# tensorlayer/TLXCV

Hardware: AMD Instinct MI355X
Metric: images/sec fwd (higher is better)
Workload: dtype f16; 1 GPU; ResNet-50 fp16 forward, 224x224, batch 256 per GPU (BASELINE configs[1]); global_batch=256, per_gpu_batch=256, weights=seeded random (tlxcv_amd.seeded, seed 1), parallelism=single GPU, launch=hipGraph replay of the forward

## Files before the change

tlxcv_amd/csrc/block_seam.hip:

```cpp
#include "kernel_util.h"
#include <stdio.h>
#include "block_seam.h"
#include <type_traits>
#ifdef TLXMI_TUNING
#define TLXMI_DBG_NT(x) (x)
#else
#define TLXMI_DBG_NT(x) (false)
#endif

namespace tlxmi {

static __device__ __forceinline__ int bs_f1(int r) { return ((r >> 1) & 1) | (((r >> 4) & 3) << 1); }
static __device__ __forceinline__ int bs_f2(int r) { return (((r >> 1) & 1) << 2) | ((r >> 5) & 1); }

static __device__ __forceinline__ unsigned bs_pkrelu(unsigned v) {
    unsigned r;
    asm("v_pk_max_f16 %0, %1, 0" : "=v"(r) : "v"(v));
    return r;
}
static __device__ __forceinline__ u32x2 bs_bn_skip_relu4(f32x4 acc, f32x4 sc, f32x4 sh, half4v skip) {
    f32x2 t0 = f32x2{__builtin_fmaf(acc[0], sc[0], (float)skip[0]), __builtin_fmaf(acc[1], sc[1], (float)skip[1])};
    f32x2 t1 = f32x2{__builtin_fmaf(acc[2], sc[2], (float)skip[2]), __builtin_fmaf(acc[3], sc[3], (float)skip[3])};
    t0 += f32x2{sh[0], sh[1]};
    t1 += f32x2{sh[2], sh[3]};
// ... 240 lines not shown
        for (int tt = 0; tt < T2; ++tt) {
            if (TLXMI_DBG(a, 16)) continue;
#pragma unroll
            for (int s = 0; s < 2; ++s) {
                const u32x4 af = *reinterpret_cast<const u32x4*>(wb + (CB + (tt >> 2)) * PANEL + (a2off[tt & 3] ^ (s << 4)));
#pragma unroll
                for (int pw = 0; pw < PW; ++pw) acc2[tt][pw] = Mma<half_t>::run(af, yf[pw][s], acc2[tt][pw]);
            }
        }

        if (more) {
            stage_write((c + 1) & 1, st);
#pragma unroll
            for (int pw = 0; pw < PW; ++pw) { sk[pw][0] = skn[pw][0]; sk[pw][1] = skn[pw][1]; }
        }
        __syncthreads();
    }

#pragma unroll
    for (int q = 0; q < N2 / 64; ++q) {
        const float* sc = tab1 + 64 * q + 16 * g;
        const float* sh = sc + N2;
#pragma unroll
        for (int h = 0; h < 2; ++h) {
            const f32x4 s0 = *reinterpret_cast<const f32x4*>(sc + 8 * h), s1 = *reinterpret_cast<const f32x4*>(sc + 8 * h + 4);
            const f32x4 h0 = *reinterpret_cast<const f32x4*>(sh + 8 * h), h1 = *reinterpret_cast<const f32x4*>(sh + 8 * h + 4);
#pragma unroll
            for (int pw = 0; pw < PW; ++pw) {
                u32x2 o0, o1;
                if constexpr (MLP) {
                    const half8v rv = __builtin_bit_cast(half8v, buf_load16(rsrd, pok[pw] ? (pix[pw] * a.res_ld + 64 * q + 16 * g + 8 * h) * 2 : BUF_OOB));
                    o0 = bs_bn_res4(acc2[4 * q + 2 * h][pw], s0, h0, half4v{rv[0], rv[1], rv[2], rv[3]});
                    o1 = bs_bn_res4(acc2[4 * q + 2 * h + 1][pw], s1, h1, half4v{rv[4], rv[5], rv[6], rv[7]});
                } else {
                    o0 = bs_bn_relu4(acc2[4 * q + 2 * h][pw], s0, h0);
                    o1 = bs_bn_relu4(acc2[4 * q + 2 * h + 1][pw], s1, h1);
                }
                const u32x4 o = u32x4{o0[0], o0[1], o1[0], o1[1]};
                if (TLXMI_DBG(a, 4)) continue;
                if (TLXMI_DBG_NT(a.z_nt)) buf_store16<BUF_NT>(zsrd, o, pok[pw] ? (pix[pw] * a.z_ld + 64 * q + 16 * g + 8 * h) * 2 : BUF_OOB);
                else buf_store16(zsrd, o, pok[pw] ? (pix[pw] * a.z_ld + 64 * q + 16 * g + 8 * h) * 2 : BUF_OOB);
            }
        }
    }
}

template <int K1, int N2, int NW>
__global__ __launch_bounds__(64 * NW, 1) void seam_pair_kernel(const SeamArgs a) {
    static_assert(N2 % 128 == 0 && NW % 2 == 0, "pairs of waves split N2 in halves of whole 64-channel blocks");
    constexpr int NT = 64 * NW;
    constexpr int IPT = 512 / NT;
    constexpr int PW = 2;
    constexpr int KS = K1 / 32;
    constexpr int CB = K1 / 64;
    constexpr int Q2 = N2 / 64;
    constexpr int NP = CB + Q2;
    constexpr int T2H = N2 / 32;
    constexpr int PANEL = 64 * 128;
    extern __shared__ __attribute__((aligned(16))) char smem[];
    char* const wbuf = smem;
    float* const tab3 = reinterpret_cast<float*>(smem + 2 * NP * PANEL);
    float* const tab1 = tab3 + 2 * a.N1;
    char* const ybuf = reinterpret_cast<char*>(tab1 + 2 * N2);

    const int t = threadIdx.x, lane = t & 63;
    const int wid = __builtin_amdgcn_readfirstlane(t >> 6);
    const int hh = wid & 1, pp = wid >> 1;
    const int fr = lane & 15, g = lane >> 4;

    const __amdgpu_buffer_rsrc_t xsrd = buf_srd(a.x, a.x_bytes), w3srd = buf_srd(a.w3, a.w3_bytes), w1srd = buf_srd(a.w1, a.w1_bytes);
    const __amdgpu_buffer_rsrc_t rsrd = buf_srd(a.res, a.res_bytes), ysrd = buf_srd(a.y, a.y_bytes), zsrd = buf_srd(a.z, a.z_bytes);

    auto stage_load = [&](int c, u32x4 (&st)[NP][IPT]) {
#pragma unroll
        for (int k = 0; k < IPT; ++k) {
            const int idx = k * NT + t, srow = idx >> 3, sslot = idx & 7;
            const int sl1 = sslot ^ bs_f1(srow), sl2 = sslot ^ bs_f2(srow);
#pragma unroll
            for (int cb = 0; cb < CB; ++cb) st[cb][k] = buf_load16(w3srd, ((64 * c + srow) * K1 + 64 * cb + 8 * sl1) * 2);
#pragma unroll
            for (int q = 0; q < Q2; ++q) st[CB + q][k] = buf_load16(w1srd, ((64 * q + srow) * a.N1 + 64 * c + 8 * sl2) * 2);
        }
    };
    auto stage_write = [&](int buf, const u32x4 (&st)[NP][IPT]) {
#pragma unroll
        for (int j = 0; j < NP; ++j)
#pragma unroll
            for (int k = 0; k < IPT; ++k) *reinterpret_cast<u32x4*>(wbuf + (buf * NP + j) * PANEL + (k * NT + t) * 16) = st[j][k];
    };

    const int m0 = ((int)blockIdx.x * (NW / 2) + pp) * (16 * PW);
    int pix[PW];
    bool pok[PW];
#pragma unroll
    for (int pw = 0; pw < PW; ++pw) {
        pix[pw] = m0 + 16 * pw + fr;
        pok[pw] = pix[pw] < a.M;
    }
    u32x4 xf[KS][PW];
#pragma unroll
    for (int pw = 0; pw < PW; ++pw)
#pragma unroll
        for (int ks = 0; ks < KS; ++ks)
            xf[ks][pw] = buf_load16(xsrd, pok[pw] ? (pix[pw] * a.x_ld + 32 * ks + 8 * g) * 2 : BUF_OOB);
    auto skip_load = [&](int c, u32x4 (&sk)[PW]) {
#pragma unroll
        for (int pw = 0; pw < PW; ++pw) sk[pw] = buf_load16(rsrd, pok[pw] ? (pix[pw] * a.res_ld + 64 * c + 16 * g + 8 * hh) * 2 : BUF_OOB);
    };
    u32x4 sk[PW];
    skip_load(0, sk);
    {
        u32x4 st[NP][IPT];
        stage_load(0, st);
        for (int i = t; i < a.N1; i += NT) {
            tab3[i] = a.scale3 ? a.scale3[i] : 1.f;
            tab3[a.N1 + i] = a.shift3 ? a.shift3[i] : 0.f;
        }
        for (int i = t; i < N2; i += NT) {
            tab1[i] = a.scale1 ? a.scale1[i] : 1.f;
            tab1[N2 + i] = a.shift1 ? a.shift1[i] : 0.f;
        }
        stage_write(0, st);
    }
    __syncthreads();

    const int arow = 16 * (fr >> 2) + (fr & 3);
    int a1off[2], a2off[4];
#pragma unroll
    for (int e = 0; e < 2; ++e) {
        const int r = arow + 4 * (2 * hh + e);
        a1off[e] = r * 128 + ((g ^ bs_f1(r)) << 4);
    }
#pragma unroll
    for (int ci = 0; ci < 4; ++ci) {
        const int r = arow + 4 * ci;
        a2off[ci] = r * 128 + (((2 * g) ^ bs_f2(r)) << 4);
    }
    char* const ymine = ybuf + (wid * PW * 64 + lane) * 16;
    const char* const ypart = ybuf + ((wid ^ 1) * PW * 64 + lane) * 16;

    f32x4 acc2[T2H][PW];
#pragma unroll
    for (int tt = 0; tt < T2H; ++tt)
#pragma unroll
        for (int pw = 0; pw < PW; ++pw) acc2[tt][pw] = f32x4{0.f, 0.f, 0.f, 0.f};

    const int nch = a.N1 >> 6;
#pragma unroll 1
    for (int c = 0; c < nch; ++c) {
        const char* const wb = wbuf + (c & 1) * NP * PANEL;
        const bool more = c + 1 < nch;
        u32x4 st[NP][IPT], skn[PW];
        if (more) {
            stage_load(c + 1, st);
            skip_load(c + 1, skn);
        }
        f32x4 acc1[2][PW];
#pragma unroll
        for (int e = 0; e < 2; ++e) {
#pragma unroll
            for (int pw = 0; pw < PW; ++pw) acc1[e][pw] = f32x4{0.f, 0.f, 0.f, 0.f};
#pragma unroll
            for (int ks = 0; ks < KS; ++ks) {
                const u32x4 af = *reinterpret_cast<const u32x4*>(wb + (ks >> 1) * PANEL + (a1off[e] ^ ((ks & 1) << 6)));
#pragma unroll
                for (int pw = 0; pw < PW; ++pw) acc1[e][pw] = Mma<half_t>::run(af, xf[ks][pw], acc1[e][pw]);
            }
        }
        u32x4 yf[PW][2];
        {
            const float* sc = tab3 + 64 * c + 16 * g + 8 * hh;
            const float* sh = sc + a.N1;
            const f32x4 s0 = *reinterpret_cast<const f32x4*>(sc), s1 = *reinterpret_cast<const f32x4*>(sc + 4);
            const f32x4 h0 = *reinterpret_cast<const f32x4*>(sh), h1 = *reinterpret_cast<const f32x4*>(sh + 4);
#pragma unroll
            for (int pw = 0; pw < PW; ++pw) {
                const half8v rv = __builtin_bit_cast(half8v, sk[pw]);
                const u32x2 o0 = bs_bn_skip_relu4(acc1[0][pw], s0, h0, half4v{rv[0], rv[1], rv[2], rv[3]});
                const u32x2 o1 = bs_bn_skip_relu4(acc1[1][pw], s1, h1, half4v{rv[4], rv[5], rv[6], rv[7]});
                const u32x4 o = u32x4{o0[0], o0[1], o1[0], o1[1]};
                buf_store16(ysrd, o, pok[pw] ? (pix[pw] * a.y_ld + 64 * c + 16 * g + 8 * hh) * 2 : BUF_OOB);
                *reinterpret_cast<u32x4*>(ymine + pw * 1024) = o;
                if (hh == 0) yf[pw][0] = o; else yf[pw][1] = o;
            }
        }
        __syncthreads();
#pragma unroll
        for (int pw = 0; pw < PW; ++pw) {
            const u32x4 o = *reinterpret_cast<const u32x4*>(ypart + pw * 1024);
            if (hh == 0) yf[pw][1] = o; else yf[pw][0] = o;
        }
#pragma unroll
        for (int tt = 0; tt < T2H; ++tt) {
#pragma unroll
            for (int s = 0; s < 2; ++s) {
                const u32x4 af = *reinterpret_cast<const u32x4*>(wb + (CB + hh * (Q2 / 2) + (tt >> 2)) * PANEL + (a2off[tt & 3] ^ (s << 4)));
#pragma unroll
                for (int pw = 0; pw < PW; ++pw) acc2[tt][pw] = Mma<half_t>::run(af, yf[pw][s], acc2[tt][pw]);
            }
        }
        if (more) {
            stage_write((c + 1) & 1, st);
#pragma unroll
            for (int pw = 0; pw < PW; ++pw) sk[pw] = skn[pw];
        }
        __syncthreads();
    }

#pragma unroll
    for (int q = 0; q < Q2 / 2; ++q) {
        const float* sc = tab1 + 64 * (hh * (Q2 / 2) + q) + 16 * g;
        const float* sh = sc + N2;
#pragma unroll
        for (int h = 0; h < 2; ++h) {
            const f32x4 s0 = *reinterpret_cast<const f32x4*>(sc + 8 * h), s1 = *reinterpret_cast<const f32x4*>(sc + 8 * h + 4);
            const f32x4 h0 = *reinterpret_cast<const f32x4*>(sh + 8 * h), h1 = *reinterpret_cast<const f32x4*>(sh + 8 * h + 4);
#pragma unroll
            for (int pw = 0; pw < PW; ++pw) {
                const u32x2 o0 = bs_bn_relu4(acc2[4 * q + 2 * h][pw], s0, h0), o1 = bs_bn_relu4(acc2[4 * q + 2 * h + 1][pw], s1, h1);
                const u32x4 o = u32x4{o0[0], o0[1], o1[0], o1[1]};
                buf_store16(zsrd, o, pok[pw] ? (pix[pw] * a.z_ld + 64 * (hh * (Q2 / 2) + q) + 16 * g + 8 * h) * 2 : BUF_OOB);
            }
        }
    }
}

template <int K1, int N2, int NW> static int launch_seam_pair_t(const SeamArgs& a, hipStream_t st) {
    constexpr int NP = K1 / 64 + N2 / 64;
    const size_t lds = (size_t)2 * NP * 64 * 128 + (size_t)(2 * a.N1 + 2 * N2) * sizeof(float) + (size_t)NW * 2 * 1024;
    if (lds > 160 * 1024) return fail(TLXMI_ERR_UNSUPPORTED, "block_seam: %zu bytes of LDS", lds);
    const void* fn = reinterpret_cast<const void*>(&seam_pair_kernel<K1, N2, NW>);
    if (int rc = raise_lds_limit(fn, 160 * 1024, "block_seam")) return rc;
    const long grid = ((long)a.M + NW * 16 - 1) / (NW * 16);
    if (grid >= (1l << 31)) return fail(TLXMI_ERR_UNSUPPORTED, "block_seam: too many rows");
    SeamArgs b = a;
    void* args[] = {&b};
    hipError_t e = hipLaunchKernel(fn, dim3((unsigned)grid), dim3(64 * NW), args, lds, st);
    if (e != hipSuccess) return fail(TLXMI_ERR_LAUNCH, "block_seam: HIP launch failed: %s", hipGetErrorString(e));
    return TLXMI_OK;
}

template <int K1, int N2, int PW, int NW, bool PROJ = false, int WPS = 0, bool MLP = false, bool DEC = false>
static int launch_seam_t(const std::conditional_t<DEC, SeamDecArgs, SeamArgs>& a, hipStream_t st) {
    constexpr int NP = K1 / 64 + N2 / 64 + (PROJ ? K1 / 64 : 0);
    const size_t lds = (size_t)2 * NP * 64 * 128 + (size_t)(2 * a.N1 + 2 * N2 + (PROJ ? 2 * a.N1 : 0)) * sizeof(float);
    if (lds > 160 * 1024) return fail(TLXMI_ERR_UNSUPPORTED, "block_seam: %zu bytes of LDS", lds);
    const void* fn = reinterpret_cast<const void*>(&seam_kernel<K1, N2, PW, NW, PROJ, WPS, MLP, DEC>);
    if (lds > 64 * 1024)
        if (int rc = raise_lds_limit(fn, 160 * 1024, "block_seam")) return rc;
    const long grid = ((long)a.M + NW * 16 * PW - 1) / (NW * 16 * PW);
    if (grid >= (1l << 31)) return fail(TLXMI_ERR_UNSUPPORTED, "block_seam: too many rows");
#ifdef TLXMI_TUNING
    if (tune_int("TLXMI_SEAM_OCC", 0)) {
        int nb = -1;
        hipError_t oe = hipOccupancyMaxActiveBlocksPerMultiprocessor(&nb, fn, 64 * NW, lds);
        fprintf(stderr, "seam<%d,%d,%d,%d,%d>: lds %zu, grid %ld, occupancy %d workgroups / CU (%s)\n", K1, N2, PW, NW, (int)PROJ, lds, grid, nb, hipGetErrorString(oe));
    }
#endif
    auto b = a;
    void* args[] = {&b};
    hipError_t e = hipLaunchKernel(fn, dim3((unsigned)grid), dim3(64 * NW), args, lds, st);
    if (e != hipSuccess) return fail(TLXMI_ERR_LAUNCH, "block_seam: HIP launch failed: %s", hipGetErrorString(e));
    return TLXMI_OK;
}

bool block_seam_shape_ok(int K1, int N1, int N2) {
    if (N1 % 64 || N1 < 64 || N1 > 2048) return false;
    if (!((K1 == 64 && (N2 == 64 || N2 == 128)) || (K1 == 128 && (N2 == 128 || N2 == 256)) || (K1 == 256 && N2 == 256))) return false;
    const size_t lds = (size_t)2 * (K1 / 64 + N2 / 64) * 64 * 128 + (size_t)(2 * N1 + 2 * N2) * sizeof(float) + (K1 == 256 ? (size_t)8 * 2 * 1024 : 0);
    return lds <= 160 * 1024;
}

int launch_mlp_seam(const SeamArgs& a0, int K1, int N2, hipStream_t st) {
    SeamArgs b = a0;
    b.z_nt = b.y_nt = 0;
    b.debug = 0;
    if (K1 == 128 && N2 == 128) return launch_seam_t<128, 128, 2, 8, false, 0, true>(b, st);
    return fail(TLXMI_ERR_UNSUPPORTED, "mlp_seam: no instantiation for %d -> N1 -> %d channels", K1, N2);
}

int launch_block_seam(const SeamArgs& a0, int K1, int N2, hipStream_t st) {
    const int vv = (int)tune_int("TLXMI_SEAM", 0);
    const int v = vv & 1;
    SeamArgs b = a0;
    b.z_nt = (vv & 2) ? 1 : 0;
    b.y_nt = (vv & 4) ? 1 : 0;
    b.debug = (int)tune_int("TLXMI_SEAM_DBG", 0);
    const SeamArgs& a = b;
    if (a.wd) {
        if (K1 == 64 && N2 == 64) return launch_seam_t<64, 64, 2, 4, true>(a, st);
        return fail(TLXMI_ERR_UNSUPPORTED, "block_seam: the projection-shortcut form is compiled for 64 -> N1 -> 64 channels");
    }
    if (vv & 16) {
        if (K1 == 64 && N2 == 64) return launch_seam_t<64, 64, 2, 4, false, 3>(a, st);
        if (K1 == 64 && N2 == 128) return launch_seam_t<64, 128, 2, 4, false, 3>(a, st);
        if (K1 == 128 && N2 == 128) return launch_seam_t<128, 128, 2, 4, false, 2>(a, st);
    }
    if (K1 == 64 && N2 == 64) return v ? launch_seam_t<64, 64, 2, 8>(a, st) : launch_seam_t<64, 64, 2, 4>(a, st);
    if (K1 == 64 && N2 == 128) return v ? launch_seam_t<64, 128, 2, 8>(a, st) : launch_seam_t<64, 128, 2, 4>(a, st);
    if (K1 == 128 && N2 == 128) return v ? launch_seam_t<128, 128, 2, 4>(a, st) : launch_seam_t<128, 128, 2, 8>(a, st);
    if (K1 == 128 && N2 == 256) return v ? launch_seam_t<128, 256, 1, 4>(a, st) : launch_seam_t<128, 256, 1, 8>(a, st);
    if (K1 == 256 && N2 == 256) {
        if (!(vv & 32)) return launch_seam_pair_t<256, 256, 8>(a, st);
        return v ? launch_seam_t<256, 256, 1, 4>(a, st) : launch_seam_t<256, 256, 1, 8>(a, st);
    }
    return fail(TLXMI_ERR_UNSUPPORTED, "block_seam: no instantiation for %d -> N1 -> %d channels", K1, N2);
}

static bool block_seam_dec_shape_ok(int K1, int N1, int N2) {
    return ((K1 == 64 && N1 == 256 && N2 == 128) || (K1 == 128 && N1 == 512 && N2 == 256)) && block_seam_shape_ok(K1, N1, N2);
}

int launch_block_seam_dec(const SeamDecArgs& a0, int K1, int N2, hipStream_t st) {
    SeamDecArgs b = a0;
    b.z_nt = b.y_nt = 0;
    b.debug = 0;
    if (K1 == 64 && N2 == 128) return launch_seam_t<64, 128, 2, 4, false, 0, false, true>(b, st);
    if (K1 == 128 && N2 == 256) return launch_seam_t<128, 256, 1, 8, false, 0, false, true>(b, st);
    return fail(TLXMI_ERR_UNSUPPORTED, "block_seam_dec: no instantiation for %d -> N1 -> %d channels", K1, N2);
}

}

using namespace tlxmi;

extern "C" int tlxmi_bottleneck_seam_supported(int dtype, int K1, int N1, int N2) {
    return dtype == TLXMI_F16 && block_seam_shape_ok(K1, N1, N2) ? 1 : 0;
}

static int seam_impl(const tlxmi_seam_desc* d, const void* t2, const void* w3_packed, const float* scale3,
                     const float* shift3, const void* skip, void* y, const void* w1_packed, const float* scale1,
                     const float* shift1, void* t1, void* stream, const void* wd_packed, const float* scale_d, const float* shift_d) {
    TLXMI_REQUIRE(d && t2 && w3_packed && skip && y && w1_packed && t1, TLXMI_ERR_BAD_ARG, "bottleneck_seam: null argument");
    TLXMI_REQUIRE(d->dtype == TLXMI_F16, TLXMI_ERR_UNSUPPORTED, "bottleneck_seam: fp16 only (the fp32 parity mode runs the two convolutions)");
    TLXMI_REQUIRE(d->rows > 0 && d->K1 > 0 && d->N1 > 0 && d->N2 > 0, TLXMI_ERR_BAD_ARG, "bottleneck_seam: bad extent");
    if (!block_seam_shape_ok(d->K1, d->N1, d->N2))
        return fail(TLXMI_ERR_UNSUPPORTED, "bottleneck_seam: no kernel for %d -> %d -> %d channels", d->K1, d->N1, d->N2);
    TLXMI_REQUIRE(d->t2_ld >= d->K1 && d->skip_ld >= (wd_packed ? d->K1 : d->N1) && d->y_ld >= d->N1 && d->t1_ld >= d->N2, TLXMI_ERR_BAD_ARG, "bottleneck_seam: row stride below the channel count");
    TLXMI_REQUIRE(!wd_packed || (aligned16(wd_packed) && d->K1 == 64 && d->N2 == 64), TLXMI_ERR_UNSUPPORTED, "bottleneck_seam_proj: 64 -> N1 -> 64 channels only");
    TLXMI_REQUIRE(d->t2_ld % 8 == 0 && d->skip_ld % 8 == 0 && d->y_ld % 8 == 0 && d->t1_ld % 8 == 0 && aligned16(t2) && aligned16(skip) && aligned16(y) &&
                      aligned16(t1) && aligned16(w3_packed) && aligned16(w1_packed),
                  TLXMI_ERR_ALIGNMENT, "bottleneck_seam: rows must be whole 16-byte chunks");
    TLXMI_REQUIRE(d->act == TLXMI_ACT_RELU, TLXMI_ERR_UNSUPPORTED, "bottleneck_seam: ReLU after both convolutions only");
    const long long rows = d->rows;
    const long long big = (1ll << 31);
    TLXMI_REQUIRE(rows * d->t2_ld * 2 < big && rows * d->skip_ld * 2 < big && rows * d->y_ld * 2 < big && rows * d->t1_ld * 2 < big && rows < big,
                  TLXMI_ERR_UNSUPPORTED, "bottleneck_seam: a tensor exceeds the 2 GiB the 32-bit buffer offsets address");
    SeamArgs a;
    a.x = (const char*)t2; a.w3 = (const char*)w3_packed; a.res = (const char*)skip; a.w1 = (const char*)w1_packed;
    a.y = (char*)y; a.z = (char*)t1;
    a.scale3 = scale3; a.shift3 = shift3; a.scale1 = scale1; a.shift1 = shift1;
    a.M = (int)rows; a.N1 = d->N1;
    a.x_ld = d->t2_ld; a.res_ld = d->skip_ld; a.y_ld = d->y_ld; a.z_ld = d->t1_ld;
    a.x_bytes = (unsigned)(rows * d->t2_ld * 2); a.res_bytes = (unsigned)(rows * d->skip_ld * 2);
    a.y_bytes = (unsigned)(rows * d->y_ld * 2); a.z_bytes = (unsigned)(rows * d->t1_ld * 2);
    a.wd = (const char*)wd_packed; a.scale_d = scale_d; a.shift_d = shift_d;
    a.wd_bytes = wd_packed ? (unsigned)(((size_t)(d->N1 + 127) / 128 * 128) * (size_t)d->K1 * 2) : 0u;
    a.w3_bytes = (unsigned)(((size_t)(d->N1 + 127) / 128 * 128) * (size_t)d->K1 * 2);
    a.w1_bytes = (unsigned)(((size_t)(d->N2 + 127) / 128 * 128) * (size_t)d->N1 * 2);
    const int rc = launch_block_seam(a, d->K1, d->N2, as_stream(stream));
    if (rc != TLXMI_OK) return rc;
    return check_launch("bottleneck_seam");
}

extern "C" int tlxmi_bottleneck_seam(const tlxmi_seam_desc* d, const void* t2, const void* w3_packed, const float* scale3,
                                     const float* shift3, const void* skip, void* y, const void* w1_packed, const float* scale1,
                                     const float* shift1, void* t1, void* stream) {
    return seam_impl(d, t2, w3_packed, scale3, shift3, skip, y, w1_packed, scale1, shift1, t1, stream, nullptr, nullptr, nullptr);
}

extern "C" int tlxmi_bottleneck_seam_proj(const tlxmi_seam_desc* d, const void* t2, const void* w3_packed, const float* scale3,
                                          const float* shift3, const void* x, const void* wd_packed, const float* scale_d,
                                          const float* shift_d, void* y, const void* w1_packed, const float* scale1,
                                          const float* shift1, void* t1, void* stream) {
    TLXMI_REQUIRE(wd_packed, TLXMI_ERR_BAD_ARG, "bottleneck_seam_proj: null shortcut filter");
    return seam_impl(d, t2, w3_packed, scale3, shift3, x, y, w1_packed, scale1, shift1, t1, stream, wd_packed, scale_d, shift_d);
}

static long long seam_dec_rows(long long rows, int H, int W) { return rows / ((long long)H * W) * ((H + 1) / 2) * ((W + 1) / 2); }

extern "C" int tlxmi_bottleneck_seam_dec_supported(int dtype, int K1, int N1, int N2, int64_t rows, int H, int W) {
    if (dtype != TLXMI_F16 || !block_seam_dec_shape_ok(K1, N1, N2) || rows <= 0 || H <= 0 || W <= 0) return 0;
    const long long big = (1ll << 31), hw = (long long)H * W;
    if (hw >= big || rows % hw) return 0;
    return rows * K1 * 2 < big && rows * N1 * 2 < big && rows * N2 * 2 < big && seam_dec_rows(rows, H, W) * N1 * 2 < big ? 1 : 0;
}

extern "C" int tlxmi_bottleneck_seam_dec(const tlxmi_seam_desc* d, int H, int W, const void* t2, const void* w3_packed, const float* scale3,
                                         const float* shift3, const void* skip, void* y, const void* w1_packed, const float* scale1,
                                         const float* shift1, void* t1, void* stream) {
    TLXMI_REQUIRE(d && t2 && w3_packed && skip && y && w1_packed && t1, TLXMI_ERR_BAD_ARG, "bottleneck_seam_dec: null argument");
    TLXMI_REQUIRE(d->dtype == TLXMI_F16, TLXMI_ERR_UNSUPPORTED, "bottleneck_seam_dec: fp16 only");
    TLXMI_REQUIRE(d->rows > 0 && d->K1 > 0 && d->N1 > 0 && d->N2 > 0 && H > 0 && W > 0, TLXMI_ERR_BAD_ARG, "bottleneck_seam_dec: bad extent");
    if (!block_seam_dec_shape_ok(d->K1, d->N1, d->N2))
        return fail(TLXMI_ERR_UNSUPPORTED, "bottleneck_seam_dec: no kernel for %d -> %d -> %d channels", d->K1, d->N1, d->N2);
    const long long big = (1ll << 31), rows = d->rows, hw = (long long)H * W;
    TLXMI_REQUIRE(hw < big && rows % hw == 0, TLXMI_ERR_BAD_ARG, "bottleneck_seam_dec: rows is not a whole number of H x W images");
    TLXMI_REQUIRE(d->t2_ld >= d->K1 && d->skip_ld >= d->N1 && d->y_ld >= d->N1 && d->t1_ld >= d->N2, TLXMI_ERR_BAD_ARG, "bottleneck_seam_dec: row stride below the channel count");
    TLXMI_REQUIRE(d->t2_ld % 8 == 0 && d->skip_ld % 8 == 0 && d->y_ld % 8 == 0 && d->t1_ld % 8 == 0 && aligned16(t2) && aligned16(skip) && aligned16(y) &&
                      aligned16(t1) && aligned16(w3_packed) && aligned16(w1_packed),
                  TLXMI_ERR_ALIGNMENT, "bottleneck_seam_dec: rows must be whole 16-byte chunks");
    TLXMI_REQUIRE(d->act == TLXMI_ACT_RELU, TLXMI_ERR_UNSUPPORTED, "bottleneck_seam_dec: ReLU after both convolutions only");
    const long long yrows = seam_dec_rows(rows, H, W);
    TLXMI_REQUIRE(rows * d->t2_ld * 2 < big && rows * d->skip_ld * 2 < big && yrows * d->y_ld * 2 < big && rows * d->t1_ld * 2 < big,
                  TLXMI_ERR_UNSUPPORTED, "bottleneck_seam_dec: a tensor exceeds the 2 GiB the 32-bit buffer offsets address");
    SeamDecArgs a;
    a.x = (const char*)t2; a.w3 = (const char*)w3_packed; a.res = (const char*)skip; a.w1 = (const char*)w1_packed;
    a.y = (char*)y; a.z = (char*)t1;
    a.scale3 = scale3; a.shift3 = shift3; a.scale1 = scale1; a.shift1 = shift1;
    a.M = (int)rows; a.N1 = d->N1;
    a.x_ld = d->t2_ld; a.res_ld = d->skip_ld; a.y_ld = d->y_ld; a.z_ld = d->t1_ld;
    a.x_bytes = (unsigned)(rows * d->t2_ld * 2); a.res_bytes = (unsigned)(rows * d->skip_ld * 2);
    a.y_bytes = (unsigned)(yrows * d->y_ld * 2); a.z_bytes = (unsigned)(rows * d->t1_ld * 2);
    a.wd = nullptr; a.scale_d = a.shift_d = nullptr; a.wd_bytes = 0;
    a.w3_bytes = (unsigned)(((size_t)(d->N1 + 127) / 128 * 128) * (size_t)d->K1 * 2);
    a.w1_bytes = (unsigned)(((size_t)(d->N2 + 127) / 128 * 128) * (size_t)d->N1 * 2);
    a.y_nt = a.z_nt = 0; a.debug = 0;
    a.HW = (int)hw; a.W = W;
    const int rc = launch_block_seam_dec(a, d->K1, d->N2, as_stream(stream));
    if (rc != TLXMI_OK) return rc;
    return check_launch("bottleneck_seam_dec");
}

extern "C" int tlxmi_mlp_seam_supported(int dtype, int K, int hidden, int N) {
    return (dtype == TLXMI_F16 && K == 128 && N == 128 && hidden % 64 == 0 && hidden >= 64 && hidden <= 2048 && block_seam_shape_ok(K, hidden, N)) ? 1 : 0;
}

extern "C" int tlxmi_mlp_seam(int dtype, int64_t rows, int K, int hidden, int N, const void* x, int x_ld, const void* w1_packed, const float* bias1,
                              const void* w2_packed, const float* bias2, const void* res, int res_ld, void* out, int out_ld, void* stream) {
    TLXMI_REQUIRE(x && w1_packed && w2_packed && res && out, TLXMI_ERR_BAD_ARG, "mlp_seam: null argument");
    if (!tlxmi_mlp_seam_supported(dtype, K, hidden, N)) return fail(TLXMI_ERR_UNSUPPORTED, "mlp_seam: no kernel for %d -> %d -> %d", K, hidden, N);
    TLXMI_REQUIRE(rows > 0 && x_ld >= K && res_ld >= N && out_ld >= N, TLXMI_ERR_BAD_ARG, "mlp_seam: bad extent");
    TLXMI_REQUIRE(x_ld % 8 == 0 && res_ld % 8 == 0 && out_ld % 8 == 0 && aligned16(x) && aligned16(res) && aligned16(out) && aligned16(w1_packed) && aligned16(w2_packed),
                  TLXMI_ERR_ALIGNMENT, "mlp_seam: rows must be whole 16-byte chunks");
    const long long big = (1ll << 31);
    TLXMI_REQUIRE(rows * x_ld * 2 < big && rows * res_ld * 2 < big && rows * out_ld * 2 < big, TLXMI_ERR_UNSUPPORTED, "mlp_seam: a tensor exceeds 2 GiB");
    SeamArgs a;
    a.x = (const char*)x; a.w3 = (const char*)w1_packed; a.res = (const char*)res; a.w1 = (const char*)w2_packed;
    a.y = nullptr; a.z = (char*)out;
    a.scale3 = nullptr; a.shift3 = bias1; a.scale1 = nullptr; a.shift1 = bias2;
    a.M = (int)rows; a.N1 = hidden;
    a.x_ld = x_ld; a.res_ld = res_ld; a.y_ld = 0; a.z_ld = out_ld;
    a.x_bytes = (unsigned)(rows * x_ld * 2); a.res_bytes = (unsigned)(rows * res_ld * 2); a.y_bytes = 0; a.z_bytes = (unsigned)(rows * out_ld * 2);
    a.wd = nullptr; a.scale_d = a.shift_d = nullptr; a.wd_bytes = 0;
    a.w3_bytes = (unsigned)(((size_t)(hidden + 127) / 128 * 128) * (size_t)K * 2);
    a.w1_bytes = (unsigned)(((size_t)(N + 127) / 128 * 128) * (size_t)hidden * 2);
    a.y_nt = a.z_nt = 0; a.debug = 0;
    const int rc = launch_mlp_seam(a, K, N, as_stream(stream));
    if (rc != TLXMI_OK) return rc;
    return check_launch("mlp_seam");
}
```

tlxcv_amd/models/classification/resnet.py:

```python
import torch

from ... import engine as E
from ...tlx import nn
from ...tlx import FlattenReshape
from ...tlx.nn import as_nhwc, from_nhwc

__all__ = ['resnet18', 'resnet34', 'resnet50', 'resnet101', 'resnet152', 'wide_resnet50_2', 'wide_resnet101_2',
           'ResNet', 'BasicBlock', 'BottleneckBlock']

_HE = nn.initializers.HeNormal()


def _conv(cin, cout, k, stride=1, padding=0, dilation=1, groups=1, data_format='channels_first'):
    return nn.GroupConv2d(in_channels=cin, out_channels=cout, kernel_size=k, stride=stride, padding=padding,
                          dilation=dilation, n_group=groups, b_init=(), W_init=_HE, data_format=data_format)


class BasicBlock(nn.Module):
    expansion = 1

    def __init__(self, in_channels, out_channels, stride=1, downsample=None, groups=1, base_width=64, dilation=1,
                 batch_norm=None, data_format='channels_first'):
        super().__init__()
        if batch_norm is None:
            batch_norm = nn.BatchNorm2d
        if dilation > 1:
            raise NotImplementedError('Dilation > 1 not supported in BasicBlock')
        self.conv1 = _conv(in_channels, out_channels, 3, stride, 1, data_format=data_format)
        self.bn1 = batch_norm(num_features=out_channels, data_format=data_format)
        self.relu = nn.ReLU()
        self.conv2 = _conv(out_channels, out_channels, 3, 1, 1, data_format=data_format)
        self.bn2 = batch_norm(num_features=out_channels, data_format=data_format)
        self.downsample = downsample
        self.stride = stride
        self.data_format = data_format

    def forward_nhwc(self, v):
        identity = v
        out = self.conv1.run_nhwc(v, self.bn1, E.ACT_RELU)
        if self.downsample is not None:
            identity = self.downsample[0].run_nhwc(v, self.downsample[1])
        return self.conv2.run_nhwc(out, self.bn2, E.ACT_RELU, res=identity)

    def forward(self, x):
        return from_nhwc(self.forward_nhwc(as_nhwc(x, self.data_format)), self.data_format)


class BottleneckBlock(nn.Module):
    expansion = 4
    proj_fold_bit = 7

    def __init__(self, in_channels, out_channels, stride=1, downsample=None, groups=1, base_width=64, dilation=1,
                 batch_norm=None, data_format='channels_first'):
        super().__init__()
        if batch_norm is None:
            batch_norm = nn.BatchNorm2d
        width = int(out_channels * (base_width / 64.0)) * groups
        self.conv1 = _conv(in_channels, width, 1, data_format=data_format)
        self.bn1 = batch_norm(num_features=width, data_format=data_format)
        self.conv2 = _conv(width, width, 3, stride, dilation, dilation, groups, data_format=data_format)
        self.bn2 = batch_norm(num_features=width, data_format=data_format)
        self.conv3 = _conv(width, out_channels * self.expansion, 1, data_format=data_format)
        self.bn3 = batch_norm(num_features=out_channels * self.expansion, data_format=data_format)
        self.relu = nn.ReLU()
        self.downsample = downsample
        self.stride = stride
        self.data_format = data_format

    def forward_nhwc(self, v):
        identity = v
        out = self.conv1.run_nhwc(v, self.bn1, E.ACT_RELU)
        out = self.conv2.run_nhwc(out, self.bn2, E.ACT_RELU)
        if self.downsample is not None:
            identity = self.downsample[0].run_nhwc(v, self.downsample[1])
        return self.conv3.run_nhwc(out, self.bn3, E.ACT_RELU, res=identity)

    def forward(self, x):
        return from_nhwc(self.forward_nhwc(as_nhwc(x, self.data_format)), self.data_format)

    def run_head(self, v, t1=None):
        out = t1 if t1 is not None else self.conv1.run_nhwc(v, self.bn1, E.ACT_RELU)
        return self.conv2.run_nhwc(out, self.bn2, E.ACT_RELU)

    def shortcut(self, v):
        return v if self.downsample is None else self.downsample[0].run_nhwc(v, self.downsample[1])

    def finish(self, out, identity):
        return self.conv3.run_nhwc(out, self.bn3, E.ACT_RELU, res=identity)

    def folded_filter(self):
        c3, cd, bnd = self.conv3, self.downsample[0], self.downsample[1]
        dt = E.precision()

        def build():
            s3, h3 = self.bn3.folded(None)
            sd, hd = bnd.folded(None)
            w3 = E._f32(c3.filters).reshape(c3.out_channels, c3.in_channels) * s3[:, None]
            wd = E._f32(cd.filters).reshape(cd.out_channels, cd.in_channels) * sd[:, None]
            return E.PackedFilter(torch.cat([w3, wd], dim=1), dt), h3 + hd
        return c3._cached(("projfold", id(cd), id(self.bn3), id(bnd)), build, deps=(cd, self.bn3, bnd))

    def fold_stride(self, out_shape, v_shape):
        ds = self.downsample
        if ds is None or E.precision() != torch.float16 or not (E.option_value("proj_fold") & self.proj_fold_bit):
            return None
        if len(ds) != 2 or not isinstance(ds[0], nn.GroupConv2d) or not isinstance(ds[1], nn.BatchNorm2d):
            return None
        if any(getattr(m, "act", None) is not None for m in (self.bn3, ds[1], self.conv3, ds[0])):
            return None
        c3, cd = self.conv3, ds[0]
        plain = lambda c: (c.kernel_size == (1, 1) and c.padding == (0, 0) and c.dilation == (1, 1) and c.n_group == 1
                           and c.biases is None and not c.same)
        if (not plain(c3) or not plain(cd) or c3.stride != (1, 1) or cd.stride not in ((1, 1), (2, 2)) or cd.out_channels != c3.out_channels
                or c3.in_channels % 64 or cd.in_channels % 64 or c3.out_channels % 8
                or out_shape[-1] != c3.in_channels or v_shape[-1] != cd.in_channels):
            return None
        stride = 1 if cd.stride == (2, 2) and tuple(v_shape[1:3]) == tuple(out_shape[1:3]) else cd.stride[0]
        pk, _ = self.folded_filter()
        return stride if E.conv1x1_proj_shapes_supported(out_shape, v_shape, pk, stride) else None

    def finish_folded(self, out, v):
        if out.dtype != E.precision() or v.dtype != out.dtype or not out.is_contiguous() or not v.is_contiguous():
            return None
        stride = self.fold_stride(out.shape, v.shape)
        if stride is None:
            return None
        pk, shift = self.folded_filter()
        return E.conv1x1_proj(out, v, pk, stride, shift=shift, act=E.ACT_RELU)

    def reads_input_at_stride2_only(self, v_shape):
        ds, c2 = self.downsample, self.conv2
        if ds is None or len(ds) != 2 or getattr(ds[0], "stride", None) != (2, 2) or c2.same:
            return False
        N, H, W, ch = v_shape
        ext = lambda n, i: (n + 2 * c2.padding[i] - c2.dilation[i] * (c2.kernel_size[i] - 1) - 1) // c2.stride[i] + 1
        out_shape = (N, ext(H, 0), ext(W, 1), c2.out_channels)
        return self.fold_stride(out_shape, (N, (H + 1) // 2, (W + 1) // 2, ch)) == 1

    def seam_with(self, nxt, out, v, y_stride2=False):
        c3, c1 = self.conv3, nxt.conv1
        dt = E.precision()
        if (not E.option("seams") or dt != torch.float16 or c3.n_group != 1 or c1.n_group != 1 or c1.kernel_size != (1, 1) or c1.stride != (1, 1)
                or c1.padding != (0, 0) or c3.biases is not None or c1.biases is not None
                or not E.bottleneck_seam_supported(c3.in_channels, c3.out_channels, c1.out_channels, dt)
                or (c3.in_channels >= 256 and not E.option("seam256"))):
            return None
        n_img = out.shape[0]
        if n_img < 12 or (c3.in_channels >= 256 and (n_img < 96 or n_img > 192)):
            return None
        pk3 = c3._cached("pk", lambda: E.PackedFilter(c3.filters, dt))
        pk1 = c1._cached("pk", lambda: E.PackedFilter(c1.filters, dt))
        s3, h3 = c3._cached(("bn", id(self.bn3)), lambda: self.bn3.folded(None), deps=(self.bn3,))
        s1, h1 = c1._cached(("bn", id(nxt.bn1)), lambda: nxt.bn1.folded(None), deps=(nxt.bn1,))
        if self.downsample is None:
            N, H, W, _ = out.shape
            dec = y_stride2 and E.bottleneck_seam_dec_supported(c3.in_channels, c3.out_channels, c1.out_channels, N * H * W, H, W, dt)
            return E.bottleneck_seam(out, pk3, s3, h3, v, pk1, s1, h1, y_stride2=dec)
        cd, bnd = self.downsample[0], self.downsample[1]
        if (cd.kernel_size == (1, 1) and cd.stride == (1, 1) and cd.padding == (0, 0) and cd.n_group == 1 and cd.biases is None
                and c3.in_channels == 64 and c1.out_channels == 64 and cd.in_channels == 64 and v.shape[-1] == 64):
            pkd = cd._cached("pk", lambda: E.PackedFilter(cd.filters, dt))
            sd, hd = cd._cached(("bn", id(bnd)), lambda: bnd.folded(None), deps=(bnd,))
            return E.bottleneck_seam(out, pk3, s3, h3, v, pk1, s1, h1, proj=(pkd, sd, hd))
        return E.bottleneck_seam(out, pk3, s3, h3, self.shortcut(v), pk1, s1, h1)


def run_bottleneck_chain(blocks, v):
    t1 = None
    for i, blk in enumerate(blocks):
        v, t1 = bottleneck_step(blk, blocks[i + 1] if i + 1 < len(blocks) else None, v, t1)
    return v


def bottleneck_step(blk, nxt, v, t1=None):
    out = blk.run_head(v, t1)
    folded = blk.finish_folded(out, v)
    if folded is not None:
        return folded, None
    if t1 is not None and v.shape[1:3] != t1.shape[1:3]:
        raise RuntimeError("bottleneck_step: the folded shortcut launch was refused after a decimated seam")
    dec = (isinstance(nxt, BottleneckBlock) and E.option("seam_decimate")
           and nxt.reads_input_at_stride2_only(tuple(out.shape[:3]) + (blk.conv3.out_channels,)))
    fused = blk.seam_with(nxt, out, v, y_stride2=dec) if isinstance(nxt, BottleneckBlock) else None
    if fused is not None:
        return fused
    return blk.finish(out, blk.shortcut(v)), None


class ResNet(nn.Module):

    def __init__(self, block, depth=50, width=64, num_classes=1000, with_pool=True, groups=1,
                 data_format='channels_first', name=None):
        super().__init__(name=name)
        layer_cfg = {18: [2, 2, 2, 2], 34: [3, 4, 6, 3], 50: [3, 4, 6, 3], 101: [3, 4, 23, 3], 152: [3, 8, 36, 3]}
        layers = layer_cfg[depth]
        self.groups = groups
        self.base_width = width
        self.num_classes = num_classes
        self.with_pool = with_pool
        self.in_channels = 64
        self.dilation = 1
        self.data_format = data_format
        self.conv1 = _conv(3, self.in_channels, 7, 2, 3, data_format=data_format)
        self.bn1 = nn.BatchNorm2d(num_features=self.in_channels, data_format=data_format)
        self.relu = nn.ReLU()
        self.maxpool = nn.MaxPool2d(kernel_size=3, stride=2, padding=1, data_format=data_format)
        self.layer1 = self._make_layer(block, 64, layers[0], data_format=data_format)
        self.layer2 = self._make_layer(block, 128, layers[1], stride=2, data_format=data_format)
        self.layer3 = self._make_layer(block, 256, layers[2], stride=2, data_format=data_format)
        self.layer4 = self._make_layer(block, 512, layers[3], stride=2, data_format=data_format)
        if block is BottleneckBlock:
            self.layer1[0].proj_fold_bit = 0
            for bit, layer in ((1, self.layer2), (2, self.layer3), (4, self.layer4)):
                layer[0].proj_fold_bit = bit
        if with_pool:
            self.avgpool = nn.AdaptiveAvgPool2d((1, 1), data_format=data_format)
        self.flatten = FlattenReshape()
        if num_classes > 0:
            self.fc = nn.Linear(in_features=512 * block.expansion, out_features=num_classes)

    def _make_layer(self, block, out_channels, blocks, stride=1, dilate=False, data_format='channels_first'):
        batch_norm = nn.BatchNorm2d
        downsample = None
        previous_dilation = self.dilation
        if dilate:
            self.dilation *= stride
            stride = 1
        if stride != 1 or self.in_channels != out_channels * block.expansion:
            downsample = nn.Sequential([
                _conv(self.in_channels, out_channels * block.expansion, 1, stride, data_format=data_format),
                batch_norm(num_features=out_channels * block.expansion, data_format=data_format)])
        layers = [block(self.in_channels, out_channels, stride, downsample, self.groups, self.base_width,
                        previous_dilation, batch_norm, data_format=data_format)]
        self.in_channels = out_channels * block.expansion
        for _ in range(1, blocks):
            layers.append(block(self.in_channels, out_channels, groups=self.groups, base_width=self.base_width,
                                batch_norm=batch_norm, data_format=data_format))
        return nn.Sequential(layers)

    @E.two_streams(96, plan="half")
    def forward(self, x):
        if (self.data_format == 'channels_first' and x.shape[2] % 2 == 0 and x.shape[3] % 2 == 0
                and not x.permute(0, 2, 3, 1).is_contiguous()):
            v = self.conv1.run_stem(x, 2, self.bn1, E.ACT_RELU, maxpool=self.maxpool)
        else:
            v = self.maxpool.run_nhwc(self.conv1.run_nhwc(as_nhwc(x, self.data_format), self.bn1, E.ACT_RELU))
        blocks = [blk for layer in (self.layer1, self.layer2, self.layer3, self.layer4) for blk in layer]
        if all(isinstance(b, BottleneckBlock) for b in blocks):
            v = run_bottleneck_chain(blocks, v)
        else:
            for blk in blocks:
                v = blk.forward_nhwc(v)
        if self.with_pool:
            v = E.global_avgpool(v)
            if self.num_classes > 0:
                return self.fc.run(v)
            N, Cc = v.shape
            return v.view(N, 1, 1, Cc) if self.data_format == 'channels_last' else v.view(N, Cc, 1, 1)
        y = from_nhwc(v, self.data_format)
        if self.num_classes > 0:
            return self.fc(self.flatten(y.contiguous()))
        return y


def _resnet(arch, Block, depth, pretrained, **kwargs):
    if pretrained:
        raise NotImplementedError("pretrained weights are not bundled; use model.load_weights(...)")
    return ResNet(Block, depth, name=arch, **kwargs)


def resnet18(pretrained=False, **kwargs):
    return _resnet('resnet18', BasicBlock, 18, pretrained, **kwargs)


def resnet34(pretrained=False, **kwargs):
    return _resnet('resnet34', BasicBlock, 34, pretrained, **kwargs)


def resnet50(pretrained=False, **kwargs):
    return _resnet('resnet50', BottleneckBlock, 50, pretrained, **kwargs)


def resnet101(pretrained=False, **kwargs):
    return _resnet('resnet101', BottleneckBlock, 101, pretrained, **kwargs)


def resnet152(pretrained=False, **kwargs):
    return _resnet('resnet152', BottleneckBlock, 152, pretrained, **kwargs)


def wide_resnet50_2(pretrained=False, **kwargs):
    return _resnet('wide_resnet50_2', BottleneckBlock, 50, pretrained, width=128, **kwargs)


def wide_resnet101_2(pretrained=False, **kwargs):
    return _resnet('wide_resnet101_2', BottleneckBlock, 101, pretrained, width=128, **kwargs)
```

Before: 80470 images/sec.

## Add antiphase two-group seam pair kernel and widen 256-channel seam batch range

Adds a new 8-wave seam kernel for the 256->N1->256 bottleneck seam. The waves are split into two groups of four that alternate between MMA phases and epilogue/DMA phases, with direct-to-LDS weight staging and a register ring of fragment prefetches. This is meant to overlap matrix-core work with the BN/skip epilogue and memory traffic. It also widens the batch range that enables the 256-channel seam from 96-192 to 48-256 images, so the batch-256 benchmark now takes the fused seam path where before it did not. In exchange it adds heavier barrier choreography, and the fused path is untested at this batch size.

```diff
diff --git a/tlxcv_amd/csrc/block_seam.hip b/tlxcv_amd/csrc/block_seam.hip
--- a/tlxcv_amd/csrc/block_seam.hip
+++ b/tlxcv_amd/csrc/block_seam.hip
@@ -416,14 +416,15 @@
         const bool more = c + 1 < nch;
         u32x4 st[NP][IPT], skn[PW];
         if (more) {
-            stage_load(c + 1, st);
-            skip_load(c + 1, skn);
+            if (!TLXMI_DBG(a, 8)) stage_load(c + 1, st);
+            if (!TLXMI_DBG(a, 2)) skip_load(c + 1, skn);
         }
         f32x4 acc1[2][PW];
 #pragma unroll
         for (int e = 0; e < 2; ++e) {
 #pragma unroll
             for (int pw = 0; pw < PW; ++pw) acc1[e][pw] = f32x4{0.f, 0.f, 0.f, 0.f};
+            if (TLXMI_DBG(a, 16)) continue;
 #pragma unroll
             for (int ks = 0; ks < KS; ++ks) {
                 const u32x4 af = *reinterpret_cast<const u32x4*>(wb + (ks >> 1) * PANEL + (a1off[e] ^ ((ks & 1) << 6)));
@@ -443,19 +444,20 @@
                 const u32x2 o0 = bs_bn_skip_relu4(acc1[0][pw], s0, h0, half4v{rv[0], rv[1], rv[2], rv[3]});
                 const u32x2 o1 = bs_bn_skip_relu4(acc1[1][pw], s1, h1, half4v{rv[4], rv[5], rv[6], rv[7]});
                 const u32x4 o = u32x4{o0[0], o0[1], o1[0], o1[1]};
-                buf_store16(ysrd, o, pok[pw] ? (pix[pw] * a.y_ld + 64 * c + 16 * g + 8 * hh) * 2 : BUF_OOB);
-                *reinterpret_cast<u32x4*>(ymine + pw * 1024) = o;
+                if (!TLXMI_DBG(a, 1)) buf_store16(ysrd, o, pok[pw] ? (pix[pw] * a.y_ld + 64 * c + 16 * g + 8 * hh) * 2 : BUF_OOB);
+                if (!TLXMI_DBG(a, 32)) *reinterpret_cast<u32x4*>(ymine + pw * 1024) = o;
                 if (hh == 0) yf[pw][0] = o; else yf[pw][1] = o;
             }
         }
         __syncthreads();
 #pragma unroll
         for (int pw = 0; pw < PW; ++pw) {
-            const u32x4 o = *reinterpret_cast<const u32x4*>(ypart + pw * 1024);
+            const u32x4 o = TLXMI_DBG(a, 32) ? (hh == 0 ? yf[pw][0] : yf[pw][1]) : *reinterpret_cast<const u32x4*>(ypart + pw * 1024);
             if (hh == 0) yf[pw][1] = o; else yf[pw][0] = o;
         }
 #pragma unroll
         for (int tt = 0; tt < T2H; ++tt) {
+            if (TLXMI_DBG(a, 16)) continue;
 #pragma unroll
             for (int s = 0; s < 2; ++s) {
                 const u32x4 af = *reinterpret_cast<const u32x4*>(wb + (CB + hh * (Q2 / 2) + (tt >> 2)) * PANEL + (a2off[tt & 3] ^ (s << 4)));
@@ -489,11 +491,250 @@
     }
 }
 
-template <int K1, int N2, int NW> static int launch_seam_pair_t(const SeamArgs& a, hipStream_t st) {
+template <int K1, int N2>
+__global__ __launch_bounds__(512, 1) void seam_pair_ap_kernel(const SeamArgs a) {
+    static_assert(N2 % 128 == 0, "pairs of waves split N2 in halves of whole 64-channel blocks");
+    constexpr int NW = 8, GT = 256;
+    constexpr int PW = 2;
+    constexpr int KS = K1 / 32;
+    constexpr int CB = K1 / 64;
+    constexpr int Q2 = N2 / 64;
+    constexpr int NP = CB + Q2;
+    constexpr int SP = CB > Q2 ? CB : Q2;
+    constexpr int T2H = N2 / 32;
+    constexpr int PANEL = 64 * 128;
+    extern __shared__ __attribute__((aligned(16))) char smem[];
+    char* const wbuf = smem;
+    float* const tab3 = reinterpret_cast<float*>(smem + 2 * NP * PANEL);
+    float* const tab1 = tab3 + 2 * a.N1;
+    char* const ybuf = reinterpret_cast<char*>(tab1 + 2 * N2);
+
+    const int t = threadIdx.x, lane = t & 63, tg = t & (GT - 1);
+    const int wid = __builtin_amdgcn_readfirstlane(t >> 6);
+    const int hh = wid & 1, pp = wid >> 1, grp = wid >> 2;
+    const int fr = lane & 15, g = lane >> 4;
+    const int nch = a.N1 >> 6;
+
+    const __amdgpu_buffer_rsrc_t xsrd = buf_srd(a.x, a.x_bytes), w3srd = buf_srd(a.w3, a.w3_bytes);
+    const __amdgpu_buffer_rsrc_t rsrd = buf_srd(a.res, a.res_bytes), ysrd = buf_srd(a.y, a.y_bytes), zsrd = buf_srd(a.z, a.z_bytes);
+
+    static_assert(CB == Q2, "both filter halves of a step are the same number of panels");
+    const int wq = wid & 3;
+    const __amdgpu_buffer_rsrc_t ssrd = buf_srd(grp == 0 ? a.w1 : a.w3, grp == 0 ? a.w1_bytes : a.w3_bytes);
+    const int sstep = grp == 0 ? 128 : 64 * K1 * 2, spanel = grp == 0 ? 64 * a.N1 * 2 : 128;
+    int soff[2];
+#pragma unroll
+    for (int k = 0; k < 2; ++k) {
+        const int idx = k * GT + tg, srow = idx >> 3, sslot = idx & 7;
+        soff[k] = grp == 0 ? (srow * a.N1 + 8 * (sslot ^ bs_f2(srow))) * 2 : ((128 + srow) * K1 + 8 * (sslot ^ bs_f1(srow))) * 2;
+    }
+    auto stage_dma = [&](int c, int dead) __attribute__((always_inline)) {
+        char* const dst = wbuf + (grp == 0 ? (((c + 1) & 1) * NP + CB) : ((c & 1) * NP)) * PANEL + wq * 1024;
+#pragma unroll
+        for (int j = 0; j < SP; ++j)
+#pragma unroll
+            for (int k = 0; k < 2; ++k) buf_dma16(ssrd, dst + j * PANEL + k * (GT * 16), (soff[k] + j * spanel + c * sstep) | dead);
+    };
+    auto phase_barrier = [&]() {
+        __builtin_amdgcn_sched_barrier(0);
+        asm volatile("s_waitcnt lgkmcnt(0)" ::: "memory");
+        __builtin_amdgcn_s_barrier();
+        __builtin_amdgcn_sched_barrier(0);
+    };
+
+    const int m0 = ((int)blockIdx.x * (NW / 2) + pp) * (16 * PW);
+    int pix[PW];
+    bool pok[PW];
+#pragma unroll
+    for (int pw = 0; pw < PW; ++pw) {
+        pix[pw] = m0 + 16 * pw + fr;
+        pok[pw] = pix[pw] < a.M;
+    }
+    u32x4 xf[KS][PW];
+#pragma unroll
+    for (int pw = 0; pw < PW; ++pw)
+#pragma unroll
+        for (int ks = 0; ks < KS; ++ks)
+            xf[ks][pw] = buf_load16(xsrd, pok[pw] ? (pix[pw] * a.x_ld + 32 * ks + 8 * g) * 2 : BUF_OOB);
+    auto skip_load = [&](int c, u32x4 (&sk)[PW], int dead) {
+#pragma unroll
+        for (int pw = 0; pw < PW; ++pw) sk[pw] = buf_load16(rsrd, pok[pw] ? ((pix[pw] * a.res_ld + 64 * c + 16 * g + 8 * hh) * 2) | dead : BUF_OOB);
+    };
+    u32x4 sk[PW];
+    skip_load(0, sk, 0);
+#pragma unroll
+    for (int k = 0; k < 2; ++k) {
+        const int idx = k * GT + tg, srow = idx >> 3, sl1 = (idx & 7) ^ bs_f1(srow);
+#pragma unroll
+        for (int j = 0; j < CB; ++j)
+            buf_dma16(w3srd, wbuf + (grp * NP + j) * PANEL + k * (GT * 16) + wq * 1024, ((64 * grp + srow) * K1 + 64 * j + 8 * sl1) * 2);
+    }
+    for (int i = t; i < a.N1; i += 64 * NW) {
+        tab3[i] = a.scale3 ? a.scale3[i] : 1.f;
+        tab3[a.N1 + i] = a.shift3 ? a.shift3[i] : 0.f;
+    }
+    for (int i = t; i < N2; i += 64 * NW) {
+        tab1[i] = a.scale1 ? a.scale1[i] : 1.f;
+        tab1[N2 + i] = a.shift1 ? a.shift1[i] : 0.f;
+    }
+    wait_vmcnt<0>();
+    __syncthreads();
+
+    const int arow = 16 * (fr >> 2) + (fr & 3);
+    int a1off[2], a2off[4];
+#pragma unroll
+    for (int e = 0; e < 2; ++e) {
+        const int r = arow + 4 * (2 * hh + e);
+        a1off[e] = r * 128 + ((g ^ bs_f1(r)) << 4);
+    }
+#pragma unroll
+    for (int ci = 0; ci < 4; ++ci) {
+        const int r = arow + 4 * ci;
+        a2off[ci] = r * 128 + (((2 * g) ^ bs_f2(r)) << 4);
+    }
+    char* const ymine = ybuf + (wid * PW * 64 + lane) * 16;
+    const char* const ypart = ybuf + ((wid ^ 1) * PW * 64 + lane) * 16;
+
+    f32x4 acc2[T2H][PW];
+#pragma unroll
+    for (int tt = 0; tt < T2H; ++tt)
+#pragma unroll
+        for (int pw = 0; pw < PW; ++pw) acc2[tt][pw] = f32x4{0.f, 0.f, 0.f, 0.f};
+    f32x4 acc1[2][PW];
+    u32x4 yown[PW], ypar[PW];
+#pragma unroll
+    for (int pw = 0; pw < PW; ++pw) yown[pw] = ypar[pw] = u32x4{0u, 0u, 0u, 0u};
+
+    auto m_phase = [&](int c, auto grp_t, auto first_t, auto last_t) __attribute__((always_inline)) {
+        constexpr int GRP = decltype(grp_t)::value;
+        constexpr bool FIRST = decltype(first_t)::value, LAST = decltype(last_t)::value;
+        const char* const wb = wbuf + (c & 1) * NP * PANEL;
+        if constexpr (GRP == 0 && !LAST) stage_dma(c, (TLXMI_DBG(a, 8) && !FIRST) ? BUF_OOB : 0);
+        if constexpr (!FIRST) {
+            if (!TLXMI_DBG(a, 32)) {
+#pragma unroll
+                for (int pw = 0; pw < PW; ++pw) ypar[pw] = *reinterpret_cast<const u32x4*>(ypart + pw * 1024);
+            }
+        }
+        if constexpr (!LAST) {
+#pragma unroll
+            for (int e = 0; e < 2; ++e)
+#pragma unroll
+                for (int pw = 0; pw < PW; ++pw) acc1[e][pw] = f32x4{0.f, 0.f, 0.f, 0.f};
+        }
+        constexpr int FD = 5;
+        constexpr int NF1 = LAST ? 0 : 2 * KS, NF2 = FIRST ? 0 : 2 * T2H, NF = NF1 + NF2;
+        auto frag = [&](int i) __attribute__((always_inline)) {
+            if (i < NF1) return *reinterpret_cast<const u32x4*>(wb + (i >> 2) * PANEL + (a1off[i & 1] ^ (((i >> 1) & 1) << 6)));
+            const int s = (i - NF1) / T2H, tt = (i - NF1) % T2H;
+            return *reinterpret_cast<const u32x4*>(wb + (CB + hh * (Q2 / 2) + (tt >> 2)) * PANEL + (a2off[tt & 3] ^ (s << 4)));
+        };
+        if (!TLXMI_DBG(a, 16)) {
+            u32x4 ring[FD], yk[2][PW];
+#pragma unroll
+            for (int i = 0; i < FD; ++i) ring[i] = frag(i);
+            __builtin_amdgcn_sched_barrier(0);
+            __builtin_amdgcn_s_setprio(1);
+#pragma unroll
+            for (int i = 0; i < NF; ++i) {
+                if constexpr (!FIRST) {
+                    if (i == NF1) {
+#pragma unroll
+                        for (int pw = 0; pw < PW; ++pw) {
+                            yk[0][pw] = hh == 0 ? yown[pw] : ypar[pw];
+                            yk[1][pw] = hh == 0 ? ypar[pw] : yown[pw];
+                        }
+                    }
+                }
+                const u32x4 af = ring[i % FD];
+                if (i < NF1) {
+#pragma unroll
+                    for (int pw = 0; pw < PW; ++pw) acc1[i & 1][pw] = Mma<half_t>::run(af, xf[i >> 1][pw], acc1[i & 1][pw]);
+                } else {
+#pragma unroll
+                    for (int pw = 0; pw < PW; ++pw) acc2[(i - NF1) % T2H][pw] = Mma<half_t>::run(af, yk[(i - NF1) / T2H][pw], acc2[(i - NF1) % T2H][pw]);
+                }
+                if (i + FD < NF) ring[i % FD] = frag(i + FD);
+                __builtin_amdgcn_sched_barrier(0);
+            }
+            __builtin_amdgcn_s_setprio(0);
+        }
+        if constexpr (GRP == 1 && !FIRST) wait_vmcnt<4>();
+        phase_barrier();
+    };
+    auto n_phase = [&](int c, auto grp_t) __attribute__((always_inline)) {
+        constexpr int GRP = decltype(grp_t)::value;
+        if constexpr (GRP == 1) {
+            stage_dma(c, (c + 2 < nch && !TLXMI_DBG(a, 8)) ? 0 : BUF_OOB);
+            __builtin_amdgcn_sched_barrier(0);
+        }
+        {
+            const float* sc = tab3 + 64 * c + 16 * g + 8 * hh;
+            const float* sh = sc + a.N1;
+            const f32x4 s0 = *reinterpret_cast<const f32x4*>(sc), s1 = *reinterpret_cast<const f32x4*>(sc + 4);
+            const f32x4 h0 = *reinterpret_cast<const f32x4*>(sh), h1 = *reinterpret_cast<const f32x4*>(sh + 4);
+            u32x4 o[PW];
+#pragma unroll
+            for (int pw = 0; pw < PW; ++pw) {
+                const half8v rv = __builtin_bit_cast(half8v, sk[pw]);
+                const u32x2 o0 = bs_bn_skip_relu4(acc1[0][pw], s0, h0, half4v{rv[0], rv[1], rv[2], rv[3]});
+                const u32x2 o1 = bs_bn_skip_relu4(acc1[1][pw], s1, h1, half4v{rv[4], rv[5], rv[6], rv[7]});
+                o[pw] = u32x4{o0[0], o0[1], o1[0], o1[1]};
+                if (!TLXMI_DBG(a, 32)) *reinterpret_cast<u32x4*>(ymine + pw * 1024) = o[pw];
+                yown[pw] = o[pw];
+            }
+            skip_load(c + 1, sk, (c + 1 < nch && !TLXMI_DBG(a, 2)) ? 0 : BUF_OOB);
+            if (!TLXMI_DBG(a, 1)) {
+#pragma unroll
+                for (int pw = 0; pw < PW; ++pw) buf_store16(ysrd, o[pw], pok[pw] ? (pix[pw] * a.y_ld + 64 * c + 16 * g + 8 * hh) * 2 : BUF_OOB);
+            }
+        }
+        if constexpr (GRP == 0) wait_vmcnt<4>();
+        phase_barrier();
+    };
+    auto run = [&](auto grp_t) __attribute__((always_inline)) {
+        if constexpr (decltype(grp_t)::value == 1) phase_barrier();
+        m_phase(0, grp_t, std::true_type{}, std::false_type{});
+        n_phase(0, grp_t);
+#pragma unroll 1
+        for (int c = 1; c < nch; ++c) {
+            m_phase(c, grp_t, std::false_type{}, std::false_type{});
+            n_phase(c, grp_t);
+        }
+        m_phase(nch, grp_t, std::false_type{}, std::true_type{});
+    };
+    if (grp == 0) run(std::integral_constant<int, 0>{});
+    else run(std::integral_constant<int, 1>{});
+
+#pragma unroll
+    for (int q = 0; q < Q2 / 2; ++q) {
+        const float* sc = tab1 + 64 * (hh * (Q2 / 2) + q) + 16 * g;
+        const float* sh = sc + N2;
+#pragma unroll
+        for (int h = 0; h < 2; ++h) {
+            const f32x4 s0 = *reinterpret_cast<const f32x4*>(sc + 8 * h), s1 = *reinterpret_cast<const f32x4*>(sc + 8 * h + 4);
+            const f32x4 h0 = *reinterpret_cast<const f32x4*>(sh + 8 * h), h1 = *reinterpret_cast<const f32x4*>(sh + 8 * h + 4);
+#pragma unroll
+            for (int pw = 0; pw < PW; ++pw) {
+                const u32x2 o0 = bs_bn_relu4(acc2[4 * q + 2 * h][pw], s0, h0), o1 = bs_bn_relu4(acc2[4 * q + 2 * h + 1][pw], s1, h1);
+                const u32x4 o = u32x4{o0[0], o0[1], o1[0], o1[1]};
+                buf_store16(zsrd, o, pok[pw] ? (pix[pw] * a.z_ld + 64 * (hh * (Q2 / 2) + q) + 16 * g + 8 * h) * 2 : BUF_OOB);
+            }
+        }
+    }
+    if (grp == 0) phase_barrier();
+}
+
+constexpr bool SEAM_PAIR_ANTIPHASE = true;
+
+template <int K1, int N2, int NW, bool AP> static int launch_seam_pair_t(const SeamArgs& a, hipStream_t st) {
+    static_assert(!AP || NW == 8, "the antiphase form is two groups of four waves");
     constexpr int NP = K1 / 64 + N2 / 64;
     const size_t lds = (size_t)2 * NP * 64 * 128 + (size_t)(2 * a.N1 + 2 * N2) * sizeof(float) + (size_t)NW * 2 * 1024;
     if (lds > 160 * 1024) return fail(TLXMI_ERR_UNSUPPORTED, "block_seam: %zu bytes of LDS", lds);
-    const void* fn = reinterpret_cast<const void*>(&seam_pair_kernel<K1, N2, NW>);
+    const void* fn;
+    if constexpr (AP) fn = reinterpret_cast<const void*>(&seam_pair_ap_kernel<K1, N2>);
+    else fn = reinterpret_cast<const void*>(&seam_pair_kernel<K1, N2, NW>);
     if (int rc = raise_lds_limit(fn, 160 * 1024, "block_seam")) return rc;
     const long grid = ((long)a.M + NW * 16 - 1) / (NW * 16);
     if (grid >= (1l << 31)) return fail(TLXMI_ERR_UNSUPPORTED, "block_seam: too many rows");
@@ -565,7 +806,10 @@
     if (K1 == 128 && N2 == 128) return v ? launch_seam_t<128, 128, 2, 4>(a, st) : launch_seam_t<128, 128, 2, 8>(a, st);
     if (K1 == 128 && N2 == 256) return v ? launch_seam_t<128, 256, 1, 4>(a, st) : launch_seam_t<128, 256, 1, 8>(a, st);
     if (K1 == 256 && N2 == 256) {
-        if (!(vv & 32)) return launch_seam_pair_t<256, 256, 8>(a, st);
+#ifdef TLXMI_TUNING
+        if (vv & 64) return launch_seam_pair_t<256, 256, 8, !SEAM_PAIR_ANTIPHASE>(a, st);
+#endif
+        if (!(vv & 32)) return launch_seam_pair_t<256, 256, 8, SEAM_PAIR_ANTIPHASE>(a, st);
         return v ? launch_seam_t<256, 256, 1, 4>(a, st) : launch_seam_t<256, 256, 1, 8>(a, st);
     }
     return fail(TLXMI_ERR_UNSUPPORTED, "block_seam: no instantiation for %d -> N1 -> %d channels", K1, N2);
diff --git a/tlxcv_amd/models/classification/resnet.py b/tlxcv_amd/models/classification/resnet.py
--- a/tlxcv_amd/models/classification/resnet.py
+++ b/tlxcv_amd/models/classification/resnet.py
@@ -9,6 +9,8 @@
            'ResNet', 'BasicBlock', 'BottleneckBlock']
 
 _HE = nn.initializers.HeNormal()
+
+SEAM14_IMAGES = (48, 256)
 
 
 def _conv(cin, cout, k, stride=1, padding=0, dilation=1, groups=1, data_format='channels_first'):
@@ -146,7 +148,7 @@
                 or (c3.in_channels >= 256 and not E.option("seam256"))):
             return None
         n_img = out.shape[0]
-        if n_img < 12 or (c3.in_channels >= 256 and (n_img < 96 or n_img > 192)):
+        if n_img < 12 or (c3.in_channels >= 256 and not SEAM14_IMAGES[0] <= n_img <= SEAM14_IMAGES[1]):
             return None
         pk3 = c3._cached("pk", lambda: E.PackedFilter(c3.filters, dt))
         pk1 = c1._cached("pk", lambda: E.PackedFilter(c1.filters, dt))
```

Result: faster. 81930 images/sec, median of 6 (+1.8%).
